# FriedFeid/Video-Depth-Anything

Measured on AMD Instinct MI355X. Metric: depth frames/sec at 32x518x518, ViT-L fp16, 1/2/4/8 MI355X, higher is better.
Workload: dtype fp16; 1 GPU; VideoDepthAnything.forward vitl 1x32x3x518x518 per GPU; encoder=vitl, frames_per_clip=32, H=518, W=518, clips_per_gpu=1, parallelism=clip-parallel dp1, ranks=1, depth_gather_to_rank0=False, hip_graph=False, clips_in_flight=2

## Files before the change

include/vda.h:

```cpp
#ifndef VDA_H
#define VDA_H

#include <stdint.h>

#ifdef __cplusplus
extern "C" {
#endif

enum {
  VDA_ACT_NONE = 0,
  VDA_ACT_GELU = 1,
  VDA_ACT_GEGLU = 2,
  VDA_ACT_RELU = 3,
  VDA_ACT_SWIGLU = 4
};

enum {
  VDA_STORE_ROWS = 0,
  VDA_STORE_PIXEL_SHUFFLE = 1
};

typedef struct vda_epilogue {
  const float* bias;
  const float* rowbias;
  int32_t rdiv, rmod;
  const float* gamma;
  const void* res;
  int64_t ldres;
  const void* res2;
  int64_t ldres2;
  int32_t act;
  int32_t store;
  int32_t ps_k, ps_cout, ps_hin, ps_win;
  const float* ln_stats;
  const float* ln_colsum;
  int32_t ln_parts;
  float ln_eps;
  float* stats_out;
  int32_t res2_h, res2_w;
  int32_t* sched;
  int32_t drop_period;
  const float* bias9;
} vda_epilogue;

const char* vda_version(void);
int64_t vda_epilogue_size(void);
const char* vda_last_error(void);

int vda_gemm(const void* x, int64_t ldx, const void* w, void* y, int64_t ldy,
             int32_t M, int32_t N, int32_t K, const vda_epilogue* epi, void* stream);
int vda_gemm_check(int64_t ldx, int64_t ldy, int32_t M, int32_t N, int32_t K, const vda_epilogue* epi);

int vda_conv2d(const void* x, const void* w, void* y, int32_t BT, int32_t H, int32_t W,
               int32_t Cin, int32_t Cout, int32_t ks, int32_t stride, int32_t pad,
               int32_t pre_relu, int32_t up_h, int32_t up_w, const vda_epilogue* epi,
               void* ws, int64_t ws_bytes, void* stream);
int64_t vda_conv2d_workspace(int32_t BT, int32_t H, int32_t W, int32_t Cin, int32_t Cout, int32_t ks,
                             int32_t stride, int32_t pad);
int vda_conv2d_res2_upsample_ok(int32_t BT, int32_t H, int32_t W, int32_t Cin, int32_t Cout, int32_t ks,
                                int32_t stride, int32_t pad);
int vda_conv2d_bias9_ok(int32_t BT, int32_t H, int32_t W, int32_t Cin, int32_t Cout, int32_t up_h, int32_t up_w);

int vda_subpixel_conv(const void* x, const void* w, const float* bias9, void* y, int32_t BT, int32_t h, int32_t w_,
                      int32_t Cin, int32_t Cout, int32_t s, void* ws, int64_t ws_bytes, void* stream);
int64_t vda_subpixel_conv_workspace(int32_t BT, int32_t h, int32_t w_, int32_t Cin, int32_t s);
int vda_subpixel_conv_check(int32_t BT, int32_t h, int32_t w_, int32_t Cin, int32_t Cout, int32_t s);

int vda_layernorm(const void* x, int64_t ldx, void* y, const float* gamma, const float* beta,
                  int32_t rows, int32_t C, float eps, int32_t skip_period, void* stream);

int vda_row_stats(const void* x, int64_t ldx, float* stats, int32_t rows, int32_t C, float eps,
                  void* stream);

int vda_groupnorm(const void* x, void* y, const float* gamma, const float* beta, int32_t F,
                  int32_t S, int32_t C, int32_t groups, float eps, float* ws, void* stream);
int64_t vda_groupnorm_workspace(int32_t F, int32_t S, int32_t C, int32_t groups);

int vda_groupnorm_linear(const void* x, const float* gamma, const float* beta, int32_t F, int32_t S,
                         int32_t C, int32_t groups, float eps, const void* w, const float* bias, void* y,
                         int32_t N, float* stats_out, void* ws, int64_t ws_bytes, void* stream);
int64_t vda_groupnorm_linear_workspace(int32_t F, int32_t S, int32_t C, int32_t groups, int32_t N);
int vda_groupnorm_linear_fused(int32_t C, int32_t groups, int32_t N);

int vda_spatial_attention(const void* qkv, void* out, int32_t B, int32_t N, int32_t H,
                          int32_t D, float scale, void* stream);

int vda_temporal_attention(const void* qkv, void* out, int32_t B, int32_t T, int32_t S,
                           int32_t H, int32_t D, float scale, float rope_theta, void* stream);

int vda_upsample_bilinear(const void* x, void* y, int32_t BT, int32_t H, int32_t W, int32_t C,
                          int32_t Ho, int32_t Wo, void* stream);

int vda_patch_im2col(const float* img, void* a, int32_t BT, int32_t H, int32_t W, int32_t Kp,
                     void* stream);

int vda_depth_head(const void* x, const void* w1, const float* b1, const float* w2,
                   const float* b2, float* depth, void* ws, int32_t BT, int32_t Hin, int32_t Win,
                   int32_t C, int32_t Ho, int32_t Wo, void* stream);
int64_t vda_depth_head_workspace(int32_t BT, int32_t Hin, int32_t Win, int32_t C, int32_t Ho, int32_t Wo);

int vda_preprocess_frames(const void* frames, float* out, int32_t N, int32_t h, int32_t w, int32_t H,
                          int32_t W, const float* mean, const float* std, void* stream);

int vda_depth_resize(const float* depth, float* out, int32_t N, int32_t H, int32_t W, int32_t ho,
                     int32_t wo, void* stream);

int64_t vda_scale_shift_workspace(int64_t n);
int vda_scale_shift(const float* pred, const float* target, const uint8_t* mask, int64_t n, double* sums,
                    float* ss, void* ws, int64_t ws_bytes, void* stream);

int vda_depth_align(const float* src, int32_t F, int32_t H, int32_t W, int32_t ho, int32_t wo, const float* ss,
                    int32_t clip, const float* pre, const float* w_pre, const float* w_post, float* out,
                    void* stream);

int64_t vda_depth_eval_workspace(int32_t F, int64_t S);
int vda_depth_eval_fit(const float* pred, const float* gt, const uint8_t* valid, int32_t F, int64_t S,
                       int32_t per_frame, double* sums, float* ss, void* ws, int64_t ws_bytes, void* stream);
int vda_depth_eval_metrics(const float* pred, const float* gt, const uint8_t* valid, int32_t F, int64_t S,
                           const float* ss, int32_t ss_per_frame, float max_depth, float* aligned,
                           double* frame_sums, double* total, void* ws, int64_t ws_bytes, void* stream);

enum {
  VDA_VIS_INDEX = 0,
  VDA_VIS_HWC = 1,
  VDA_VIS_PLANAR444 = 2,
  VDA_VIS_PLANAR420 = 3
};
int64_t vda_depth_range_workspace(int64_t n);
int vda_depth_range(const float* depth, int64_t n, float* range, void* ws, int64_t ws_bytes, void* stream);
int64_t vda_depth_colorize_bytes(int32_t F, int32_t H, int32_t W, int32_t layout);
int vda_depth_colorize(const float* depth, int32_t F, int32_t H, int32_t W, const float* range,
                       const uint8_t* lut, int32_t layout, uint8_t* out, void* stream);

enum {
  VDA_TILE_RGB = 0,
  VDA_TILE_DEPTH = 1,
  VDA_TILE_ERROR = 2,
  VDA_TILE_XT = 3
};
typedef struct vda_tile {
  int32_t kind;
  int32_t row, col;
  int32_t offset;
  int32_t frames;
  int32_t lut;
  const void* a;
  const float* b;
  const uint8_t* valid;
  const float* range;
} vda_tile;
int64_t vda_tile_size(void);
int64_t vda_depth_absdiff_range_workspace(int64_t n);
int vda_depth_absdiff_range(const float* a, const float* b, const uint8_t* valid, int64_t n, float* range, void* ws,
                            int64_t ws_bytes, void* stream);
int64_t vda_panel_compose_bytes(int32_t F, int32_t rows, int32_t cols, int32_t H, int32_t W, int32_t layout);
int vda_panel_compose(const vda_tile* tiles, int32_t ntiles, int32_t rows, int32_t cols, int32_t F, int32_t t0,
                      int32_t N, int32_t H, int32_t W, int32_t xstar, const uint8_t* lut0, const uint8_t* lut1,
                      int32_t layout, uint8_t* out, void* stream);

enum {
  VDA_YUV_420 = 0,
  VDA_YUV_422 = 1,
  VDA_YUV_444 = 2,
  VDA_YUV_MONO = 3
};
int vda_yuv_to_rgb(const uint8_t* src, int32_t N, int32_t h, int32_t w, int64_t frame_stride, int32_t chroma,
                   uint8_t* out, void* stream);
int64_t vda_preprocess_yuv_workspace(int32_t N, int32_t h, int32_t w, int32_t H, int32_t W);
int vda_preprocess_yuv(const uint8_t* src, int32_t N, int32_t h, int32_t w, int64_t frame_stride, int32_t chroma,
                       float* out, int32_t H, int32_t W, const float* mean, const float* stdv, void* ws,
                       int64_t ws_bytes, void* stream);
int32_t vda_resample_taps(int32_t in, int32_t out);
int vda_resample_tables(int32_t in, int32_t out, int32_t* k, int32_t* bounds);
int vda_yuv_downscale_ok(int32_t h, int32_t w, int32_t h2, int32_t w2);
int64_t vda_yuv_downscale_workspace(int32_t N, int32_t h, int32_t w, int32_t h2, int32_t w2);
int vda_yuv_downscale(const uint8_t* src, int32_t N, int32_t h, int32_t w, int64_t frame_stride, int32_t chroma,
                      const int32_t* kx, const int32_t* bx, const int32_t* ky, const int32_t* by, uint8_t* out,
                      int32_t h2, int32_t w2, void* ws, int64_t ws_bytes, void* stream);

int vda_gemm_f32(const float* x, int64_t ldx, const float* w, float* y, int64_t ldy,
                 int32_t M, int32_t N, int32_t K, const vda_epilogue* epi, void* stream);
int vda_conv2d_f32(const float* x, const float* w, float* y, int32_t BT, int32_t H, int32_t W,
                   int32_t Cin, int32_t Cout, int32_t ks, int32_t stride, int32_t pad,
                   int32_t pre_relu, const vda_epilogue* epi, void* stream);
int vda_layernorm_f32(const float* x, int64_t ldx, float* y, const float* gamma, const float* beta,
                      int32_t rows, int32_t C, float eps, int32_t skip_period, void* stream);
int vda_groupnorm_f32(const float* x, float* y, const float* gamma, const float* beta, int32_t F,
                      int32_t S, int32_t C, int32_t groups, float eps, void* stream);
int vda_spatial_attention_f32(const float* qkv, float* out, int32_t B, int32_t N, int32_t H,
                              int32_t D, float scale, void* stream);
int vda_temporal_attention_f32(const float* qkv, float* out, int32_t B, int32_t T, int32_t S,
                               int32_t H, int32_t D, float scale, float rope_theta, void* stream);
int vda_upsample_bilinear_f32(const float* x, float* y, int32_t BT, int32_t H, int32_t W, int32_t C,
                              int32_t Ho, int32_t Wo, void* stream);
int vda_patch_im2col_f32(const float* img, float* a, int32_t BT, int32_t H, int32_t W, int32_t Kp,
                         void* stream);
int vda_depth_head_f32(const float* x, const float* w1, const float* b1, const float* w2,
                       const float* b2, float* depth, float* ws_up, float* ws_mid, int32_t BT,
                       int32_t Hin, int32_t Win, int32_t C, int32_t Ho, int32_t Wo, void* stream);


#ifdef __cplusplus
}
#endif
#endif
```

include/vda_tune.h:

```cpp
#ifndef VDA_TUNE_H
#define VDA_TUNE_H
#include <stdint.h>
#ifdef __cplusplus
extern "C" {
#endif

int vda_debug_force_tile(int32_t cfg);
int vda_debug_gemm_sched(int32_t persist_blocks);
int vda_debug_strip_split(int32_t nsplit);
int vda_debug_hconv(int32_t mode);
int vda_debug_dconv(int32_t mode);
int vda_debug_oc1_src(int32_t mode);
int vda_debug_attn(int32_t temporal_direct);

#ifdef __cplusplus
}
#endif
#endif
```

video-depth-anything_amd/_lib.py:

```python
from __future__ import annotations

import ctypes
import os
from ctypes import c_float, c_int32, c_int64, c_void_p, POINTER

_HERE = os.path.dirname(os.path.abspath(__file__))
LIB_PATH = os.environ.get("VDA_LIB_OVERRIDE") or os.path.join(_HERE, "libvda.so")
TORCH_LIB_PATH = os.path.join(_HERE, "libvda_torch.so")
if os.environ.get("VDA_LIB_OVERRIDE"):
    _ov = os.path.join(os.path.dirname(os.path.abspath(os.environ["VDA_LIB_OVERRIDE"])), "libvda_torch.so")
    if os.path.exists(_ov):
        TORCH_LIB_PATH = _ov

EXPORTED = (
    "vda_version", "vda_epilogue_size", "vda_last_error", "vda_gemm", "vda_gemm_check", "vda_conv2d", "vda_conv2d_workspace",
    "vda_layernorm",
    "vda_conv2d_res2_upsample_ok", "vda_conv2d_bias9_ok",
    "vda_subpixel_conv", "vda_subpixel_conv_workspace", "vda_subpixel_conv_check",
    "vda_row_stats", "vda_groupnorm", "vda_groupnorm_workspace",
    "vda_groupnorm_linear", "vda_groupnorm_linear_workspace", "vda_groupnorm_linear_fused",
    "vda_spatial_attention", "vda_temporal_attention", "vda_upsample_bilinear", "vda_patch_im2col",
    "vda_depth_head", "vda_depth_head_workspace", "vda_preprocess_frames", "vda_depth_resize",
    "vda_scale_shift", "vda_scale_shift_workspace", "vda_depth_align",
    "vda_depth_eval_workspace", "vda_depth_eval_fit", "vda_depth_eval_metrics",
    "vda_depth_range_workspace", "vda_depth_range", "vda_depth_colorize_bytes", "vda_depth_colorize",
    "vda_tile_size", "vda_depth_absdiff_range_workspace", "vda_depth_absdiff_range", "vda_panel_compose_bytes",
    "vda_panel_compose",
    "vda_yuv_to_rgb", "vda_preprocess_yuv_workspace", "vda_preprocess_yuv",
    "vda_resample_taps", "vda_resample_tables", "vda_yuv_downscale_ok", "vda_yuv_downscale_workspace",
    "vda_yuv_downscale",
    "vda_gemm_f32", "vda_conv2d_f32", "vda_layernorm_f32", "vda_groupnorm_f32", "vda_spatial_attention_f32",
    "vda_temporal_attention_f32", "vda_upsample_bilinear_f32", "vda_patch_im2col_f32", "vda_depth_head_f32",
)
TUNE_EXPORTED = ("vda_debug_force_tile", "vda_debug_gemm_sched", "vda_debug_strip_split", "vda_debug_hconv",
                 "vda_debug_dconv", "vda_debug_attn", "vda_debug_oc1_src")
TUNE_LIB_PATH = os.path.join(os.path.dirname(_HERE), "build", "tune", "libvda.so")

ACT_NONE, ACT_GELU, ACT_GEGLU, ACT_RELU, ACT_SWIGLU = 0, 1, 2, 3, 4
STORE_ROWS, STORE_PIXEL_SHUFFLE = 0, 1
VIS_INDEX, VIS_HWC, VIS_PLANAR444, VIS_PLANAR420 = 0, 1, 2, 3
TILE_RGB, TILE_DEPTH, TILE_ERROR, TILE_XT = 0, 1, 2, 3
YUV_420, YUV_422, YUV_444, YUV_MONO = 0, 1, 2, 3


class VDAUnavailable(RuntimeError):
    pass


class VDAError(RuntimeError):
    pass


class Epilogue(ctypes.Structure):
    _fields_ = [
        ("bias", c_void_p), ("rowbias", c_void_p), ("rdiv", c_int32), ("rmod", c_int32),
        ("gamma", c_void_p), ("res", c_void_p), ("ldres", c_int64), ("res2", c_void_p),
        ("ldres2", c_int64), ("act", c_int32), ("store", c_int32), ("ps_k", c_int32),
        ("ps_cout", c_int32), ("ps_hin", c_int32), ("ps_win", c_int32),
        ("ln_stats", c_void_p), ("ln_colsum", c_void_p), ("ln_parts", c_int32), ("ln_eps", c_float),
        ("stats_out", c_void_p), ("res2_h", c_int32), ("res2_w", c_int32), ("sched", c_void_p),
        ("drop_period", c_int32), ("bias9", c_void_p),
    ]


class Tile(ctypes.Structure):
    _fields_ = [
        ("kind", c_int32), ("row", c_int32), ("col", c_int32), ("offset", c_int32), ("frames", c_int32),
        ("lut", c_int32), ("a", c_void_p), ("b", c_void_p), ("valid", c_void_p), ("range", c_void_p),
    ]


_lib = None
_load_error = None


def _declare(lib):
    P, I, L, F = c_void_p, c_int32, c_int64, c_float
    EP = POINTER(Epilogue)
    sig = {
        "vda_version": ([], ctypes.c_char_p),
        "vda_epilogue_size": ([], L),
        "vda_last_error": ([], ctypes.c_char_p),
        "vda_gemm": ([P, L, P, P, L, I, I, I, EP, P], I),
        "vda_gemm_check": ([L, L, I, I, I, EP], I),
        "vda_conv2d": ([P, P, P, I, I, I, I, I, I, I, I, I, I, I, EP, P, L, P], I),
        "vda_conv2d_workspace": ([I, I, I, I, I, I, I, I], L),
        "vda_conv2d_res2_upsample_ok": ([I, I, I, I, I, I, I, I], I),
        "vda_conv2d_bias9_ok": ([I, I, I, I, I, I, I], I),
        "vda_subpixel_conv": ([P, P, P, P, I, I, I, I, I, I, P, L, P], I),
        "vda_subpixel_conv_workspace": ([I, I, I, I, I], L),
        "vda_subpixel_conv_check": ([I, I, I, I, I, I], I),
        "vda_layernorm": ([P, L, P, P, P, I, I, F, I, P], I),
        "vda_row_stats": ([P, L, P, I, I, F, P], I),
        "vda_groupnorm": ([P, P, P, P, I, I, I, I, F, P, P], I),
        "vda_groupnorm_workspace": ([I, I, I, I], L),
        "vda_groupnorm_linear": ([P, P, P, I, I, I, I, F, P, P, P, I, P, P, L, P], I),
        "vda_groupnorm_linear_workspace": ([I, I, I, I, I], L),
        "vda_groupnorm_linear_fused": ([I, I, I], I),
        "vda_spatial_attention": ([P, P, I, I, I, I, F, P], I),
        "vda_temporal_attention": ([P, P, I, I, I, I, I, F, F, P], I),
        "vda_upsample_bilinear": ([P, P, I, I, I, I, I, I, P], I),
        "vda_patch_im2col": ([P, P, I, I, I, I, P], I),
        "vda_depth_head": ([P, P, P, P, P, P, P, I, I, I, I, I, I, P], I),
        "vda_depth_head_workspace": ([I, I, I, I, I, I], L),
        "vda_preprocess_frames": ([P, P, I, I, I, I, I, POINTER(F), POINTER(F), P], I),
        "vda_depth_resize": ([P, P, I, I, I, I, I, P], I),
        "vda_scale_shift_workspace": ([L], L),
        "vda_scale_shift": ([P, P, P, L, P, P, P, L, P], I),
        "vda_depth_align": ([P, I, I, I, I, I, P, I, P, POINTER(F), POINTER(F), P, P], I),
        "vda_depth_eval_workspace": ([I, L], L),
        "vda_depth_eval_fit": ([P, P, P, I, L, I, P, P, P, L, P], I),
        "vda_depth_eval_metrics": ([P, P, P, I, L, P, I, F, P, P, P, P, L, P], I),
        "vda_depth_range_workspace": ([L], L),
        "vda_depth_range": ([P, L, P, P, L, P], I),
        "vda_depth_colorize_bytes": ([I, I, I, I], L),
        "vda_depth_colorize": ([P, I, I, I, P, P, I, P, P], I),
        "vda_tile_size": ([], L),
        "vda_depth_absdiff_range_workspace": ([L], L),
        "vda_depth_absdiff_range": ([P, P, P, L, P, P, L, P], I),
        "vda_panel_compose_bytes": ([I, I, I, I, I, I], L),
        "vda_panel_compose": ([POINTER(Tile), I, I, I, I, I, I, I, I, I, P, P, I, P, P], I),
        "vda_yuv_to_rgb": ([P, I, I, I, L, I, P, P], I),
        "vda_preprocess_yuv_workspace": ([I, I, I, I, I], L),
        "vda_preprocess_yuv": ([P, I, I, I, L, I, P, I, I, POINTER(F), POINTER(F), P, L, P], I),
        "vda_resample_taps": ([I, I], I),
        "vda_resample_tables": ([I, I, P, P], I),
        "vda_yuv_downscale_ok": ([I, I, I, I], I),
        "vda_yuv_downscale_workspace": ([I, I, I, I, I], L),
        "vda_yuv_downscale": ([P, I, I, I, L, I, P, P, P, P, P, I, I, P, L, P], I),
        "vda_gemm_f32": ([P, L, P, P, L, I, I, I, EP, P], I),
        "vda_conv2d_f32": ([P, P, P, I, I, I, I, I, I, I, I, I, EP, P], I),
        "vda_layernorm_f32": ([P, L, P, P, P, I, I, F, I, P], I),
        "vda_groupnorm_f32": ([P, P, P, P, I, I, I, I, F, P], I),
        "vda_spatial_attention_f32": ([P, P, I, I, I, I, F, P], I),
        "vda_temporal_attention_f32": ([P, P, I, I, I, I, I, F, F, P], I),
        "vda_upsample_bilinear_f32": ([P, P, I, I, I, I, I, I, P], I),
        "vda_patch_im2col_f32": ([P, P, I, I, I, I, P], I),
        "vda_depth_head_f32": ([P, P, P, P, P, P, P, P, I, I, I, I, I, I, P], I),
        "vda_debug_force_tile": ([I], I),
        "vda_debug_gemm_sched": ([I], I),
        "vda_debug_strip_split": ([I], I),
        "vda_debug_hconv": ([I], I),
        "vda_debug_dconv": ([I], I),
        "vda_debug_attn": ([I], I),
        "vda_debug_oc1_src": ([I], I),
    }
    for name, (args, res) in sig.items():
        if name.startswith("vda_debug_") and not hasattr(lib, name):
            continue
        fn = getattr(lib, name)
        fn.argtypes = args
        fn.restype = res


def lib():
    global _lib, _load_error
    if _lib is not None:
        return _lib
    if _load_error is not None:
        raise VDAUnavailable(_load_error)
    if not os.path.exists(LIB_PATH):
        _load_error = f"libvda.so not found at {LIB_PATH}; run `make` (or __graft_entry__.build())"
        raise VDAUnavailable(_load_error)
    try:
        l = ctypes.CDLL(LIB_PATH)
        _declare(l)
        if l.vda_epilogue_size() != ctypes.sizeof(Epilogue):
            raise OSError(f"vda_epilogue is {l.vda_epilogue_size()} bytes in the library, {ctypes.sizeof(Epilogue)} "
                          f"in _lib.Epilogue: rebuild libvda.so or update the mirror")
        if l.vda_tile_size() != ctypes.sizeof(Tile):
            raise OSError(f"vda_tile is {l.vda_tile_size()} bytes in the library, {ctypes.sizeof(Tile)} in _lib.Tile: "
                          f"rebuild libvda.so or update the mirror")
    except OSError as e:
        _load_error = f"failed to load {LIB_PATH}: {e}"
        raise VDAUnavailable(_load_error) from e
    _lib = l
    return _lib


_torch_ops = None


def torch_ops():
    global _torch_ops
    if _torch_ops is not None:
        return _torch_ops
    lib()
    if not os.path.exists(TORCH_LIB_PATH):
        raise VDAUnavailable(f"libvda_torch.so not found at {TORCH_LIB_PATH}; run `make` (or __graft_entry__.build())")
    import torch
    try:
        torch.ops.load_library(TORCH_LIB_PATH)
    except OSError as e:
        raise VDAUnavailable(f"failed to load {TORCH_LIB_PATH}: {e}") from e
    _torch_ops = torch.ops.vda
    return _torch_ops


def check(rc: int, what: str):
    if rc != 0:
        msg = lib().vda_last_error().decode(errors="replace")
        raise VDAError(f"{what} failed (rc={rc}): {msg}")
```

video-depth-anything_amd/csrc/vda_hconv.hip:

```cpp
#include "vda_internal.h"
#include "vda_halo.h"
#include <type_traits>

namespace {

constexpr int HC_TR = 8, HC_TC = 32;
constexpr int HC_PC = HC_TC + 2;
constexpr int HC_NPIX = (HC_TR + 2) * HC_PC;
constexpr int HC_PSTR = 9;
constexpr int HC_PP = (HC_NPIX * HC_PSTR + 63) / 64;
constexpr int HC_PSLOT = HC_PP * 512;
constexpr int HC_PPW = (HC_PP + 7) / 8;
static_assert(HC_PP % 8 == 0, "the wait_vmcnt counts assume every wave issues HC_PPW patch pieces");
constexpr int HC_BK = 64;
constexpr int HC_HALF = 128 * HC_BK;
constexpr int HC_WBUF = 2 * HC_HALF;
static_assert(HC_PPW <= 9, "patch pieces are issued in the first steps of a slab");

__device__ __attribute__((aligned(64))) uint4 g_hc_zero[4];

#ifdef VDA_TS
__device__ unsigned long long g_hts[8192][6];
#define HTS(k) (hts[k] = __builtin_amdgcn_s_memrealtime())
#else
#define HTS(k) ((void)0)
#endif

__device__ __forceinline__ int hc_swz(int row, int chunk) { return row * HC_BK + ((chunk ^ ((row >> 1) & 7)) << 3); }

struct HconvArgs {
  const h16* x;
  const h16* w;
  h16* y;
  const float* bias;
  const h16* res;
  const h16* res2;
  int r2h, r2w;
  int H, W, Cin, relu_out;
  int tiles_x, tiles_y, ntiles;
};

template <bool PRE>
__global__ __launch_bounds__(512) void hconv256_kernel(HconvArgs a) {
  __shared__ __attribute__((aligned(1024))) h16 smem[2 * HC_WBUF + 2 * HC_PSLOT];
#ifdef VDA_TS
  unsigned long long hts[6];
#endif
  HTS(0);
  h16* const wsm = smem;
  h16* const psm = smem + 2 * HC_WBUF;

  int tid;
  asm volatile("v_mov_b32 %0, %1" : "=v"(tid) : "v"((int)threadIdx.x));
  const int lane = tid & 63;
  const int wave = __builtin_amdgcn_readfirstlane(tid >> 6);
  const int wm = wave & 1, wn = wave >> 1;

  int bt, y0, x0;
  {
    const int bid = blockIdx.x, nwg = a.ntiles;
    const int xcd = bid & 7, q = nwg >> 3, r = nwg & 7;
    const int t = (xcd < r ? xcd * (q + 1) : r * (q + 1) + (xcd - r) * q) + (bid >> 3);
    const int tx = t % a.tiles_x;
    const int rr = t / a.tiles_x;
    y0 = (rr % a.tiles_y) * HC_TR;
    x0 = tx * HC_TC;
    bt = rr / a.tiles_y;
  }
  const int H = a.H, W = a.W, Cin = a.Cin;
  const int K = 9 * Cin;
  const int nslab = Cin / 64;
  const int NK = 9 * nslab;
  const h16* xf0 = a.x + (long)bt * H * W * Cin;

  int poff[HC_PPW];
#pragma unroll
  for (int j = 0; j < HC_PPW; ++j) {
    const int q = wave + 8 * j;
    const int sl = q * 64 + lane;
    const int p = sl / HC_PSTR, cd = sl - p * HC_PSTR;
    const int pr = p / HC_PC, pc = p - pr * HC_PC;
    const int iy = y0 - 1 + pr, ix = x0 - 1 + pc;
    poff[j] = (q < HC_PP && p < HC_NPIX && cd < 8 && (unsigned)iy < (unsigned)H && (unsigned)ix < (unsigned)W)
                  ? (iy * W + ix) * Cin + cd * 8
                  : -1;
  }
  uint64_t zpa = (uint64_t)(uintptr_t)g_hc_zero;
  asm volatile("" : "+s"(zpa));
  const void* const zero = (const void*)(uintptr_t)zpa;
  auto patch_piece = [&](int slab, int j) {
    const int q = wave + 8 * j;
    if (q < HC_PP) {
      const void* src = poff[j] >= 0 ? (const void*)(xf0 + poff[j] + slab * 64) : zero;
      glds16(src, psm + (slab & 1) * HC_PSLOT + q * 512);
    }
  };

  auto wr_of = [&](int i) { return (wave >> 2) * 64 + i * 32 + (wave & 3) * 8 + (lane >> 3); };
  const int kch0 = ((lane & 7) ^ ((((wave & 1) << 3 | (lane >> 3)) >> 1) & 7)) * 8;
  const __amdgpu_buffer_rsrc_t wrs =
      __builtin_amdgcn_make_buffer_rsrc((void*)a.w, (short)0, (int)(256L * K * 2), 0x00020000);
  unsigned wvo[2][2];
#pragma unroll
  for (int i = 0; i < 2; ++i)
#pragma unroll
    for (int hh = 0; hh < 2; ++hh) wvo[hh][i] = (unsigned)(((hh * 128 + wr_of(i)) * K + kch0) * 2);
  auto koff = [&](int kt) {
    const int slab = kt / 9, tap = kt - slab * 9;
    return (tap * Cin + slab * 64) * 2;
  };
  auto stage_w = [&](int kt, int buf, int i) {
    const int so = koff(kt);
#pragma unroll
    for (int hh = 0; hh < 2; ++hh)
      __builtin_amdgcn_raw_ptr_buffer_load_lds(
          wrs, (VDA_LDS void*)(wsm + buf * HC_WBUF + hh * HC_HALF + (wr_of(i) - (lane >> 3)) * HC_BK), 16,
          (int)wvo[hh][i], so, 0, 0);
  };

  f4 acc[4][8];
#pragma unroll
  for (int i = 0; i < 4; ++i)
#pragma unroll
    for (int j = 0; j < 8; ++j) acc[i][j] = f4{0.f, 0.f, 0.f, 0.f};
  f4 bias_r[4];
#pragma unroll
  for (int i = 0; i < 4; ++i)
    bias_r[i] = a.bias ? *reinterpret_cast<const f4*>(a.bias + wn * 64 + i * 16 + (lane >> 4) * 4) : f4{0.f, 0.f, 0.f, 0.f};

#pragma unroll
  for (int j = 0; j < HC_PPW; ++j) patch_piece(0, j);
  stage_w(0, 0, 0);
  stage_w(0, 0, 1);
  if (NK > 1) {
    stage_w(1, 1, 1);
    wait_vmcnt<2>();
  } else {
    wait_vmcnt<0>();
  }
  __builtin_amdgcn_s_barrier();
  static_assert(HC_PP * 64 == 6 * 512, "relu pass: two passes of 3 slots per thread cover the patch exactly");
  auto relu_pass = [&](int slot, int part) {
    h8* ps = reinterpret_cast<h8*>(psm + slot * HC_PSLOT) + tid + 512 * 3 * part;
    h8 v[3];
#pragma unroll
    for (int k = 0; k < 3; ++k) v[k] = ps[512 * k];
#pragma unroll
    for (int k = 0; k < 3; ++k) ps[512 * k] = relu8(v[k]);
  };
  if (PRE) {
    relu_pass(0, 0);
    relu_pass(0, 1);
    asm volatile("s_waitcnt lgkmcnt(0)" ::: "memory");
    __builtin_amdgcn_s_barrier();
  }
  HTS(1);
  const bool lagging = wave >= 4;
  if (lagging) __builtin_amdgcn_s_barrier();

  const int frow = lane & 15, fchunk = lane >> 4;
  const int woff = (wn >> 1) * HC_HALF;
  const int wrow0 = (wn & 1) * 64;
  h8 xf[4][2], wf[2][2];
  const unsigned xlane = (unsigned)(((wm * 4 * HC_PC + frow) * HC_PSTR + fchunk) * 16);
  auto load_x = [&](const h16* ps, int toff, int qm) {
    unsigned tb;
    asm volatile("s_mov_b32 %0, %1" : "=s"(tb) : "s"((unsigned)((uintptr_t)(VDA_LDS const h16*)ps) + (unsigned)(toff * HC_PSTR * 16)));
    const VDA_LDS char* xb = reinterpret_cast<const VDA_LDS char*>((uintptr_t)(tb + xlane));
#pragma unroll
    for (int j = 0; j < 4; ++j)
#pragma unroll
      for (int ks = 0; ks < 2; ++ks)
        xf[j][ks] = *reinterpret_cast<const VDA_LDS h8*>(
            xb + ((qm * 2 + (j >> 1)) * HC_PC + (j & 1) * 16) * HC_PSTR * 16 + ks * 64);
  };
  auto load_w = [&](const h16* base, int qn) {
#pragma unroll
    for (int i = 0; i < 2; ++i)
#pragma unroll
      for (int ks = 0; ks < 2; ++ks)
        wf[i][ks] = *reinterpret_cast<const h8*>(&base[woff + hc_swz(wrow0 + qn * 32 + i * 16 + frow, ks * 4 + fchunk)]);
  };
  auto mma = [&](int qm, int qn) {
    __builtin_amdgcn_s_barrier();
    asm volatile("s_waitcnt lgkmcnt(0)" ::: "memory");
    __builtin_amdgcn_sched_barrier(0);
    __builtin_amdgcn_s_setprio(1);
#pragma unroll
    for (int ks = 0; ks < 2; ++ks)
#pragma unroll
      for (int i = 0; i < 2; ++i)
#pragma unroll
        for (int j = 0; j < 4; ++j)
          acc[qn * 2 + i][qm * 4 + j] = mfma16(wf[i][ks], xf[j][ks], acc[qn * 2 + i][qm * 4 + j]);
    __builtin_amdgcn_s_setprio(0);
    __builtin_amdgcn_sched_barrier(0);
    __builtin_amdgcn_s_barrier();
  };

  for (int slab = 0; slab < nslab; ++slab) {
    const h16* ps = psm + (slab & 1) * HC_PSLOT;
    const bool nxt = slab + 1 < nslab;
    auto step = [&](auto tap_c) {
      constexpr int tap = decltype(tap_c)::value;
      constexpr int toff = (tap / 3) * HC_PC + (tap % 3);
      const int kt = slab * 9 + tap;
      const int cb = kt & 1, nb = cb ^ 1;
      const h16* base = wsm + cb * HC_WBUF;
      const bool more1 = kt + 1 < NK, more2 = kt + 2 < NK;
      load_x(ps, toff, 0);
      load_w(base, 0);
      if (tap < HC_PPW && nxt) patch_piece(slab + 1, tap < HC_PPW ? tap : 0);
      mma(0, 0);
      load_w(base, 1);
      if (more1) stage_w(kt + 1, nb, 0);
      if (PRE && tap >= 7 && nxt) relu_pass((slab + 1) & 1, tap >= 7 ? tap - 7 : 0);
      mma(0, 1);
      load_x(ps, toff, 1);
      mma(1, 1);
      load_w(base, 0);
      if (more2) {
        stage_w(kt + 2, cb, 1);
        wait_vmcnt<2>();
      } else {
        wait_vmcnt<0>();
      }
      mma(1, 0);
    };
    step(std::integral_constant<int, 0>{}); step(std::integral_constant<int, 1>{});
    step(std::integral_constant<int, 2>{}); step(std::integral_constant<int, 3>{});
    step(std::integral_constant<int, 4>{}); step(std::integral_constant<int, 5>{});
    step(std::integral_constant<int, 6>{}); step(std::integral_constant<int, 7>{});
    step(std::integral_constant<int, 8>{});
  }
  if (!lagging) __builtin_amdgcn_s_barrier();
  HTS(2);
  __syncthreads();

  const int q = tid & 31, row0 = tid >> 5;
  const h16* l0 = smem + row0 * 256 + ((2 * q) ^ row0) * 4;
  const h16* l1 = smem + row0 * 256 + ((2 * q + 1) ^ row0) * 4;
  const long fbytes = (long)H * W * 512;
  const long fbase = (long)bt * H * W * 256;
  auto rsrc = [&](const h16* p) {
    return __builtin_amdgcn_make_buffer_rsrc((void*)(p + fbase), (short)0, (int)fbytes, 0x00020000);
  };
  const __amdgpu_buffer_rsrc_t ry = rsrc(a.y);
  auto voff = [&](int it) {
    const int yy = y0 + (it >> 1), xx = x0 + row0 + 16 * (it & 1);
    return (yy < H && xx < W) ? (unsigned)(((yy * W + xx) * 256 + q * 8) * 2) : 0x80000000u;
  };
  const bool up2 = a.r2h > 0;
  const h16* pres2 = up2 ? nullptr : a.res2;
  const int nres = (a.res ? 1 : 0) + (pres2 ? 1 : 0);
  const h16* r1p = a.res ? a.res : pres2;
  const __amdgpu_buffer_rsrc_t rr1 = rsrc(r1p ? r1p : a.y);
  const __amdgpu_buffer_rsrc_t rr2 = rsrc(pres2 ? pres2 : a.y);
  const __amdgpu_buffer_rsrc_t rs2 = __builtin_amdgcn_make_buffer_rsrc(
      (void*)((up2 ? a.res2 : a.y) + (up2 ? (long)bt * a.r2h * a.r2w * 256 : fbase)), (short)0,
      up2 ? (int)((long)a.r2h * a.r2w * 512) : (int)fbytes, 0x00020000);
  const float usy = a.r2h > 0 ? ac_scale(a.r2h, H) : 0.f, usx = a.r2w > 0 ? ac_scale(a.r2w, W) : 0.f;
  auto up_load = [&](int it, h8* t4, float& wx, float& wy) {
    const int yy = min(y0 + (it >> 1), H - 1), xx = min(x0 + row0 + 16 * (it & 1), W - 1);
    int sy0, sy1, sx0, sx1;
    ac_coord(yy, a.r2h, usy, sy0, sy1, wy);
    ac_coord(xx, a.r2w, usx, sx0, sx1, wx);
    const unsigned r0 = (unsigned)(sy0 * a.r2w), r1 = (unsigned)(sy1 * a.r2w), c8 = (unsigned)q * 16u;
    t4[0] = __builtin_bit_cast(h8, __builtin_amdgcn_raw_buffer_load_b128(rs2, (r0 + sx0) * 512u + c8, 0, 0));
    t4[1] = __builtin_bit_cast(h8, __builtin_amdgcn_raw_buffer_load_b128(rs2, (r0 + sx1) * 512u + c8, 0, 0));
    t4[2] = __builtin_bit_cast(h8, __builtin_amdgcn_raw_buffer_load_b128(rs2, (r1 + sx0) * 512u + c8, 0, 0));
    t4[3] = __builtin_bit_cast(h8, __builtin_amdgcn_raw_buffer_load_b128(rs2, (r1 + sx1) * 512u + c8, 0, 0));
  };
  constexpr int UPD = 2;
  h8 u4[UPD][4];
  float uwx[UPD], uwy[UPD];
  if (up2) {
#pragma unroll
    for (int it = 0; it < UPD; ++it) up_load(it, u4[it], uwx[it], uwy[it]);
  }
  constexpr int PD = 4;
  h8 q1[PD], q2[PD];
  if (nres >= 1) {
#pragma unroll
    for (int it = 0; it < PD; ++it) q1[it] = __builtin_bit_cast(h8, __builtin_amdgcn_raw_buffer_load_b128(rr1, voff(it), 0, 0));
  }
  if (nres >= 2) {
#pragma unroll
    for (int it = 0; it < PD; ++it) q2[it] = __builtin_bit_cast(h8, __builtin_amdgcn_raw_buffer_load_b128(rr2, voff(it), 0, 0));
  }
  const int mcol = lane & 15, nq = (lane >> 4) * 4;
#pragma unroll
  for (int i = 0; i < 4; ++i) {
    const int col = wn * 64 + i * 16 + nq;
    const f4 bv = bias_r[i];
#pragma unroll
    for (int j = 0; j < 8; ++j) {
      const int ml = wm * 128 + j * 16 + mcol;
      f4 v = acc[i][j] + bv;
      if (a.relu_out) {
#pragma unroll
        for (int r = 0; r < 4; ++r) v[r] = fmaxf(v[r], 0.f);
      }
      typedef float f2v __attribute__((ext_vector_type(2)));
      const h2 lo = __builtin_convertvector(f2v{v[0], v[1]}, h2);
      const h2 hi = __builtin_convertvector(f2v{v[2], v[3]}, h2);
      const int u = (col >> 2) ^ (ml & 15);
      *reinterpret_cast<uint2*>(&smem[ml * 256 + u * 4]) =
          make_uint2(__builtin_bit_cast(unsigned, lo), __builtin_bit_cast(unsigned, hi));
    }
  }
  __syncthreads();
  HTS(3);
#pragma unroll
  for (int it = 0; it < 16; ++it) {
    const uint2 lo = *reinterpret_cast<const uint2*>(l0 + it * 16 * 256);
    const uint2 hi = *reinterpret_cast<const uint2*>(l1 + it * 16 * 256);
    h8 t = __builtin_bit_cast(h8, make_uint4(lo.x, lo.y, hi.x, hi.y));
    const unsigned vo = voff(it);
    if (nres >= 1) {
      t += q1[it % PD];
      if (it + PD < 16) q1[it % PD] = __builtin_bit_cast(h8, __builtin_amdgcn_raw_buffer_load_b128(rr1, voff(it + PD), 0, 0));
    }
    if (nres >= 2) {
      t += q2[it % PD];
      if (it + PD < 16) q2[it % PD] = __builtin_bit_cast(h8, __builtin_amdgcn_raw_buffer_load_b128(rr2, voff(it + PD), 0, 0));
    }
    if (up2) {
      const int sl = it % UPD;
      t += bilerp8(u4[sl][0], u4[sl][1], u4[sl][2], u4[sl][3], uwx[sl], uwy[sl]);
      if (it + UPD < 16) up_load(it + UPD, u4[sl], uwx[sl], uwy[sl]);
    }
    __builtin_amdgcn_raw_buffer_store_b128(__builtin_bit_cast(u32x4, t), ry, vo, 0, 2);
  }
#ifdef VDA_TS
  HTS(4);
  asm volatile("s_waitcnt vmcnt(0)" ::: "memory");
  HTS(5);
  if (tid == 0 && blockIdx.x < 8192)
    for (int k = 0; k < 6; ++k) g_hts[blockIdx.x][k] = hts[k];
#endif
}

}

VDA_KNOB(int, g_hconv_mode, -1);

bool vda_conv_hconv_serves(int BT, int H, int W, int Cin, int Cout) {
  if (Cout != 256 || Cin % 64 != 0 || Cin <= 0 || g_hconv_mode == 0) return false;
  if ((long)BT * ((H + HC_TR - 1) / HC_TR) * ((W + HC_TC - 1) / HC_TC) > 0x7fffffffL) return false;
  if ((long)H * W * Cin >= (1L << 31) || (long)H * W * 512 >= (1L << 31)) return false;
  if (g_hconv_mode == 1) return true;
  return (long)H * W >= 64L * 64L;
}

int vda_conv_hconv(const void* x, const void* w, void* y, const float* bias, int relu_out, int pre_relu,
                   const void* res, const void* res2, int res2_h, int res2_w, int BT, int H, int W, int Cin, int Cout,
                   hipStream_t st) {
  if (!vda_conv_hconv_serves(BT, H, W, Cin, Cout)) return 1;
  HconvArgs a{};
  a.x = (const h16*)x; a.w = (const h16*)w; a.y = (h16*)y; a.bias = bias;
  a.res = (const h16*)res; a.res2 = (const h16*)res2;
  a.r2h = res2 && res2_h > 0 && res2_w > 0 ? res2_h : 0;
  a.r2w = a.r2h > 0 ? res2_w : 0;
  a.H = H; a.W = W; a.Cin = Cin; a.relu_out = relu_out;
  a.tiles_x = (W + HC_TC - 1) / HC_TC;
  a.tiles_y = (H + HC_TR - 1) / HC_TR;
  a.ntiles = BT * a.tiles_x * a.tiles_y;
  if (pre_relu)
    hipLaunchKernelGGL(hconv256_kernel<true>, dim3(a.ntiles), dim3(512), 0, st, a);
  else
    hipLaunchKernelGGL(hconv256_kernel<false>, dim3(a.ntiles), dim3(512), 0, st, a);
  VDA_LAUNCH_CHECK();
  return 0;
}

#ifdef VDA_TS
extern "C" int vda_debug_hconv_timestamps(void* host) {
  return (int)hipMemcpyFromSymbol(host, HIP_SYMBOL(g_hts), sizeof(g_hts), 0, hipMemcpyDeviceToHost);
}
#endif
#ifdef VDA_TUNING
extern "C" int vda_debug_hconv(int32_t mode) {
  g_hconv_mode = mode;
  return 0;
}
#endif
```

Baseline: 741.8 frames/s.

## Template the 256-out 3x3 conv on tile shape and pick the fewest-tile shape

The hconv256 kernel becomes a template over its output tile shape, with 8x32, 10x25 and 16x16 on a menu. A host-side chooser picks the shape that covers the feature map with the fewest tiles, which cuts edge padding waste on the 74/148/296-wide DPT maps. Tiles whose width is not a multiple of 16 need a padded LDS patch pitch, per-fragment row-crossing address fixups (bfe/mad) and a remapped epilogue pixel index. The cost is extra ALU work in the fragment loads and some extra LDS pitch on those shapes.

```diff
diff --git a/include/vda.h b/include/vda.h
--- a/include/vda.h
+++ b/include/vda.h
@@ -60,6 +60,7 @@
 int vda_conv2d_res2_upsample_ok(int32_t BT, int32_t H, int32_t W, int32_t Cin, int32_t Cout, int32_t ks,
                                 int32_t stride, int32_t pad);
 int vda_conv2d_bias9_ok(int32_t BT, int32_t H, int32_t W, int32_t Cin, int32_t Cout, int32_t up_h, int32_t up_w);
+int vda_hconv_tile_shape(int32_t H, int32_t W, int32_t* tr, int32_t* tc);
 
 int vda_subpixel_conv(const void* x, const void* w, const float* bias9, void* y, int32_t BT, int32_t h, int32_t w_,
                       int32_t Cin, int32_t Cout, int32_t s, void* ws, int64_t ws_bytes, void* stream);
diff --git a/include/vda_tune.h b/include/vda_tune.h
--- a/include/vda_tune.h
+++ b/include/vda_tune.h
@@ -9,6 +9,7 @@
 int vda_debug_gemm_sched(int32_t persist_blocks);
 int vda_debug_strip_split(int32_t nsplit);
 int vda_debug_hconv(int32_t mode);
+int vda_debug_hconv_tile(int32_t k);
 int vda_debug_dconv(int32_t mode);
 int vda_debug_oc1_src(int32_t mode);
 int vda_debug_attn(int32_t temporal_direct);
diff --git a/video-depth-anything_amd/_lib.py b/video-depth-anything_amd/_lib.py
--- a/video-depth-anything_amd/_lib.py
+++ b/video-depth-anything_amd/_lib.py
@@ -15,7 +15,7 @@
 EXPORTED = (
     "vda_version", "vda_epilogue_size", "vda_last_error", "vda_gemm", "vda_gemm_check", "vda_conv2d", "vda_conv2d_workspace",
     "vda_layernorm",
-    "vda_conv2d_res2_upsample_ok", "vda_conv2d_bias9_ok",
+    "vda_conv2d_res2_upsample_ok", "vda_conv2d_bias9_ok", "vda_hconv_tile_shape",
     "vda_subpixel_conv", "vda_subpixel_conv_workspace", "vda_subpixel_conv_check",
     "vda_row_stats", "vda_groupnorm", "vda_groupnorm_workspace",
     "vda_groupnorm_linear", "vda_groupnorm_linear_workspace", "vda_groupnorm_linear_fused",
@@ -33,7 +33,7 @@
     "vda_temporal_attention_f32", "vda_upsample_bilinear_f32", "vda_patch_im2col_f32", "vda_depth_head_f32",
 )
 TUNE_EXPORTED = ("vda_debug_force_tile", "vda_debug_gemm_sched", "vda_debug_strip_split", "vda_debug_hconv",
-                 "vda_debug_dconv", "vda_debug_attn", "vda_debug_oc1_src")
+                 "vda_debug_dconv", "vda_debug_attn", "vda_debug_oc1_src", "vda_debug_hconv_tile")
 TUNE_LIB_PATH = os.path.join(os.path.dirname(_HERE), "build", "tune", "libvda.so")
 
 ACT_NONE, ACT_GELU, ACT_GEGLU, ACT_RELU, ACT_SWIGLU = 0, 1, 2, 3, 4
@@ -74,7 +74,7 @@
 _load_error = None
 
 
-def _declare(lib):
+def _declare(lib, older=False):
     P, I, L, F = c_void_p, c_int32, c_int64, c_float
     EP = POINTER(Epilogue)
     sig = {
@@ -87,6 +87,7 @@
         "vda_conv2d_workspace": ([I, I, I, I, I, I, I, I], L),
         "vda_conv2d_res2_upsample_ok": ([I, I, I, I, I, I, I, I], I),
         "vda_conv2d_bias9_ok": ([I, I, I, I, I, I, I], I),
+        "vda_hconv_tile_shape": ([I, I, POINTER(I), POINTER(I)], I),
         "vda_subpixel_conv": ([P, P, P, P, I, I, I, I, I, I, P, L, P], I),
         "vda_subpixel_conv_workspace": ([I, I, I, I, I], L),
         "vda_subpixel_conv_check": ([I, I, I, I, I, I], I),
@@ -141,12 +142,15 @@
         "vda_debug_gemm_sched": ([I], I),
         "vda_debug_strip_split": ([I], I),
         "vda_debug_hconv": ([I], I),
+        "vda_debug_hconv_tile": ([I], I),
         "vda_debug_dconv": ([I], I),
         "vda_debug_attn": ([I], I),
         "vda_debug_oc1_src": ([I], I),
     }
     for name, (args, res) in sig.items():
         if name.startswith("vda_debug_") and not hasattr(lib, name):
+            continue
+        if older and not hasattr(lib, name):
             continue
         fn = getattr(lib, name)
         fn.argtypes = args
@@ -164,7 +168,7 @@
         raise VDAUnavailable(_load_error)
     try:
         l = ctypes.CDLL(LIB_PATH)
-        _declare(l)
+        _declare(l, older=bool(os.environ.get("VDA_LIB_OVERRIDE")))
         if l.vda_epilogue_size() != ctypes.sizeof(Epilogue):
             raise OSError(f"vda_epilogue is {l.vda_epilogue_size()} bytes in the library, {ctypes.sizeof(Epilogue)} "
                           f"in _lib.Epilogue: rebuild libvda.so or update the mirror")
diff --git a/video-depth-anything_amd/csrc/vda_hconv.hip b/video-depth-anything_amd/csrc/vda_hconv.hip
--- a/video-depth-anything_amd/csrc/vda_hconv.hip
+++ b/video-depth-anything_amd/csrc/vda_hconv.hip
@@ -4,9 +4,7 @@
 
 namespace {
 
-constexpr int HC_TR = 8, HC_TC = 32;
-constexpr int HC_PC = HC_TC + 2;
-constexpr int HC_NPIX = (HC_TR + 2) * HC_PC;
+constexpr int HC_NPIX = 340;
 constexpr int HC_PSTR = 9;
 constexpr int HC_PP = (HC_NPIX * HC_PSTR + 63) / 64;
 constexpr int HC_PSLOT = HC_PP * 512;
@@ -25,6 +23,25 @@
 #else
 #define HTS(k) ((void)0)
 #endif
+
+template <int TR, int TC>
+struct HcShape {
+  static_assert(TC >= 16, "a 16-pixel fragment crosses at most one row end");
+  static_assert(TR * TC <= 256, "one MFMA column per tile pixel");
+  static_assert((TR + 2) * (TC + 2) <= HC_NPIX, "the patch fits the slot");
+  static constexpr int PC = TC + 2;
+  static constexpr bool straight = TC % 16 == 0 && 128 % TC == 0;
+  static constexpr int RPAD = straight ? 0 : 1;
+  static constexpr int RPITCH = PC * HC_PSTR + RPAD;
+  static constexpr int ROWSH = 2 * HC_PSTR + RPAD;
+  static constexpr int pslot(int p) { return p * HC_PSTR + (p / TC) * ROWSH; }
+  static_assert((TR + 2) * RPITCH <= HC_PP * 64, "the padded patch fits the slot");
+  static_assert(pslot(255) + 2 * RPITCH + 2 * HC_PSTR + 8 <= HC_PP * 64,
+                "the last (dead) column's last tap reads inside the slot");
+};
+
+constexpr int HC_NMENU = 3;
+constexpr int HC_MENU[HC_NMENU][2] = {{8, 32}, {10, 25}, {16, 16}};
 
 __device__ __forceinline__ int hc_swz(int row, int chunk) { return row * HC_BK + ((chunk ^ ((row >> 1) & 7)) << 3); }
 
@@ -40,8 +57,9 @@
   int tiles_x, tiles_y, ntiles;
 };
 
-template <bool PRE>
+template <bool PRE, int TR, int TC>
 __global__ __launch_bounds__(512) void hconv256_kernel(HconvArgs a) {
+  using S = HcShape<TR, TC>;
   __shared__ __attribute__((aligned(1024))) h16 smem[2 * HC_WBUF + 2 * HC_PSLOT];
 #ifdef VDA_TS
   unsigned long long hts[6];
@@ -63,8 +81,8 @@
     const int t = (xcd < r ? xcd * (q + 1) : r * (q + 1) + (xcd - r) * q) + (bid >> 3);
     const int tx = t % a.tiles_x;
     const int rr = t / a.tiles_x;
-    y0 = (rr % a.tiles_y) * HC_TR;
-    x0 = tx * HC_TC;
+    y0 = (rr % a.tiles_y) * TR;
+    x0 = tx * TC;
     bt = rr / a.tiles_y;
   }
   const int H = a.H, W = a.W, Cin = a.Cin;
@@ -78,12 +96,22 @@
   for (int j = 0; j < HC_PPW; ++j) {
     const int q = wave + 8 * j;
     const int sl = q * 64 + lane;
-    const int p = sl / HC_PSTR, cd = sl - p * HC_PSTR;
-    const int pr = p / HC_PC, pc = p - pr * HC_PC;
-    const int iy = y0 - 1 + pr, ix = x0 - 1 + pc;
-    poff[j] = (q < HC_PP && p < HC_NPIX && cd < 8 && (unsigned)iy < (unsigned)H && (unsigned)ix < (unsigned)W)
-                  ? (iy * W + ix) * Cin + cd * 8
-                  : -1;
+    if constexpr (S::RPAD == 0) {
+      const int p = sl / HC_PSTR, cd = sl - p * HC_PSTR;
+      const int pr = p / S::PC, pc = p - pr * S::PC;
+      const int iy = y0 - 1 + pr, ix = x0 - 1 + pc;
+      poff[j] = (q < HC_PP && p < (TR + 2) * S::PC && cd < 8 && (unsigned)iy < (unsigned)H && (unsigned)ix < (unsigned)W)
+                    ? (iy * W + ix) * Cin + cd * 8
+                    : -1;
+    } else {
+      const int pr = (int)((unsigned)sl / (unsigned)S::RPITCH);
+      const unsigned ws = (unsigned)(sl - pr * S::RPITCH);
+      const int pc = (int)(ws / (unsigned)HC_PSTR), cd = (int)ws - pc * HC_PSTR;
+      const int iy = y0 - 1 + pr, ix = x0 - 1 + pc;
+      poff[j] = (q < HC_PP && pr < TR + 2 && pc < S::PC && cd < 8 && (unsigned)iy < (unsigned)H && (unsigned)ix < (unsigned)W)
+                    ? (iy * W + ix) * Cin + cd * 8
+                    : -1;
+    }
   }
   uint64_t zpa = (uint64_t)(uintptr_t)g_hc_zero;
   asm volatile("" : "+s"(zpa));
@@ -124,9 +152,11 @@
 #pragma unroll
     for (int j = 0; j < 8; ++j) acc[i][j] = f4{0.f, 0.f, 0.f, 0.f};
   f4 bias_r[4];
-#pragma unroll
-  for (int i = 0; i < 4; ++i)
-    bias_r[i] = a.bias ? *reinterpret_cast<const f4*>(a.bias + wn * 64 + i * 16 + (lane >> 4) * 4) : f4{0.f, 0.f, 0.f, 0.f};
+  if constexpr (S::RPAD == 0) {
+  #pragma unroll
+    for (int i = 0; i < 4; ++i)
+      bias_r[i] = a.bias ? *reinterpret_cast<const f4*>(a.bias + wn * 64 + i * 16 + (lane >> 4) * 4) : f4{0.f, 0.f, 0.f, 0.f};
+  }
 
 #pragma unroll
   for (int j = 0; j < HC_PPW; ++j) patch_piece(0, j);
@@ -162,17 +192,33 @@
   const int woff = (wn >> 1) * HC_HALF;
   const int wrow0 = (wn & 1) * 64;
   h8 xf[4][2], wf[2][2];
-  const unsigned xlane = (unsigned)(((wm * 4 * HC_PC + frow) * HC_PSTR + fchunk) * 16);
-  auto load_x = [&](const h16* ps, int toff, int qm) {
+  const unsigned xlane = S::RPAD == 0 ? (unsigned)(((wm * (S::pslot(128) / HC_PSTR) + frow) * HC_PSTR + fchunk) * 16)
+                                     : (unsigned)((wm * S::pslot(128) + frow * HC_PSTR + fchunk) * 16);
+  unsigned xrows = 0;
+  if constexpr (!S::straight) {
+#pragma unroll
+    for (int k = 0; k < 8; ++k)
+      xrows |= (unsigned)((128 * wm + 16 * k + frow) / TC - (16 * k) / TC - wm * (128 / TC)) << (2 * k);
+  }
+  auto load_x = [&](const h16* ps, int toff, auto qm_c) {
+    constexpr int qm = decltype(qm_c)::value;
     unsigned tb;
-    asm volatile("s_mov_b32 %0, %1" : "=s"(tb) : "s"((unsigned)((uintptr_t)(VDA_LDS const h16*)ps) + (unsigned)(toff * HC_PSTR * 16)));
-    const VDA_LDS char* xb = reinterpret_cast<const VDA_LDS char*>((uintptr_t)(tb + xlane));
-#pragma unroll
-    for (int j = 0; j < 4; ++j)
+    asm volatile("s_mov_b32 %0, %1" : "=s"(tb) : "s"((unsigned)((uintptr_t)(VDA_LDS const h16*)ps) + (unsigned)(toff * 16)));
+    const unsigned xq = tb + xlane;
+#pragma unroll
+    for (int j = 0; j < 4; ++j) {
+      const int k = qm * 4 + j;
+      unsigned xa = xq;
+      if constexpr (!S::straight) {
+        asm volatile("v_bfe_u32 %0, %1, %2, 2\n\tv_mad_u32_u24 %0, %0, %3, %4"
+                     : "=&v"(xa)
+                     : "v"(xrows), "i"(2 * k), "s"((unsigned)(S::ROWSH * 16)), "v"(xq));
+      }
+      const VDA_LDS char* xb = reinterpret_cast<const VDA_LDS char*>((uintptr_t)xa);
 #pragma unroll
       for (int ks = 0; ks < 2; ++ks)
-        xf[j][ks] = *reinterpret_cast<const VDA_LDS h8*>(
-            xb + ((qm * 2 + (j >> 1)) * HC_PC + (j & 1) * 16) * HC_PSTR * 16 + ks * 64);
+        xf[j][ks] = *reinterpret_cast<const VDA_LDS h8*>(xb + S::pslot(16 * k) * 16 + ks * 64);
+    }
   };
   auto load_w = [&](const h16* base, int qn) {
 #pragma unroll
@@ -203,12 +249,12 @@
     const bool nxt = slab + 1 < nslab;
     auto step = [&](auto tap_c) {
       constexpr int tap = decltype(tap_c)::value;
-      constexpr int toff = (tap / 3) * HC_PC + (tap % 3);
+      constexpr int toff = (tap / 3) * S::RPITCH + (tap % 3) * HC_PSTR;
       const int kt = slab * 9 + tap;
       const int cb = kt & 1, nb = cb ^ 1;
       const h16* base = wsm + cb * HC_WBUF;
       const bool more1 = kt + 1 < NK, more2 = kt + 2 < NK;
-      load_x(ps, toff, 0);
+      load_x(ps, toff, std::integral_constant<int, 0>{});
       load_w(base, 0);
       if (tap < HC_PPW && nxt) patch_piece(slab + 1, tap < HC_PPW ? tap : 0);
       mma(0, 0);
@@ -216,7 +262,7 @@
       if (more1) stage_w(kt + 1, nb, 0);
       if (PRE && tap >= 7 && nxt) relu_pass((slab + 1) & 1, tap >= 7 ? tap - 7 : 0);
       mma(0, 1);
-      load_x(ps, toff, 1);
+      load_x(ps, toff, std::integral_constant<int, 1>{});
       mma(1, 1);
       load_w(base, 0);
       if (more2) {
@@ -235,9 +281,27 @@
   }
   if (!lagging) __builtin_amdgcn_s_barrier();
   HTS(2);
+  if constexpr (S::RPAD != 0) {
+  #pragma unroll
+    for (int i = 0; i < 4; ++i)
+      bias_r[i] = a.bias ? *reinterpret_cast<const f4*>(a.bias + wn * 64 + i * 16 + (lane >> 4) * 4) : f4{0.f, 0.f, 0.f, 0.f};
+  }
   __syncthreads();
 
   const int q = tid & 31, row0 = tid >> 5;
+  auto tile_px = [&](int it, int& py, int& pc) {
+    const int r = (16 * it) / TC, c = (16 * it) % TC;
+    if constexpr (TC % 16 == 0) {
+      py = r;
+      pc = c;
+      return TR * TC == 256 || 16 * it < TR * TC;
+    } else {
+      const bool cross = row0 + c >= TC;
+      py = r + (cross ? 1 : 0);
+      pc = c - (cross ? TC : 0);
+      return TR * TC == 256 || row0 + 16 * it < TR * TC;
+    }
+  };
   const h16* l0 = smem + row0 * 256 + ((2 * q) ^ row0) * 4;
   const h16* l1 = smem + row0 * 256 + ((2 * q + 1) ^ row0) * 4;
   const long fbytes = (long)H * W * 512;
@@ -247,8 +311,10 @@
   };
   const __amdgpu_buffer_rsrc_t ry = rsrc(a.y);
   auto voff = [&](int it) {
-    const int yy = y0 + (it >> 1), xx = x0 + row0 + 16 * (it & 1);
-    return (yy < H && xx < W) ? (unsigned)(((yy * W + xx) * 256 + q * 8) * 2) : 0x80000000u;
+    int py, pc;
+    const bool live = tile_px(it, py, pc);
+    const int yy = y0 + py, xx = x0 + row0 + pc;
+    return (live && yy < H && xx < W) ? (unsigned)(((yy * W + xx) * 256 + q * 8) * 2) : 0x80000000u;
   };
   const bool up2 = a.r2h > 0;
   const h16* pres2 = up2 ? nullptr : a.res2;
@@ -261,7 +327,9 @@
       up2 ? (int)((long)a.r2h * a.r2w * 512) : (int)fbytes, 0x00020000);
   const float usy = a.r2h > 0 ? ac_scale(a.r2h, H) : 0.f, usx = a.r2w > 0 ? ac_scale(a.r2w, W) : 0.f;
   auto up_load = [&](int it, h8* t4, float& wx, float& wy) {
-    const int yy = min(y0 + (it >> 1), H - 1), xx = min(x0 + row0 + 16 * (it & 1), W - 1);
+    int py, pc;
+    tile_px(it, py, pc);
+    const int yy = min(y0 + py, H - 1), xx = min(x0 + row0 + pc, W - 1);
     int sy0, sy1, sx0, sx1;
     ac_coord(yy, a.r2h, usy, sy0, sy1, wy);
     ac_coord(xx, a.r2w, usx, sx0, sx1, wx);
@@ -344,13 +412,48 @@
 }
 
 VDA_KNOB(int, g_hconv_mode, -1);
+VDA_KNOB(int, g_hconv_tile, 0);
+
+static long hc_tiles(int m, int H, int W) {
+  const int tr = HC_MENU[m][0], tc = HC_MENU[m][1];
+  return (long)((H + tr - 1) / tr) * ((W + tc - 1) / tc);
+}
+
+static int hc_auto_shape(int H, int W) {
+  int best = 0;
+  for (int m = 1; m < HC_NMENU; ++m) {
+    const long t = hc_tiles(m, H, W), tb = hc_tiles(best, H, W);
+    if (t < tb || (t == tb && best != 0 && HC_MENU[m][0] * HC_MENU[m][1] > HC_MENU[best][0] * HC_MENU[best][1])) best = m;
+  }
+  return best;
+}
+
+static int hc_shape(int H, int W) { return g_hconv_tile >= 1 ? g_hconv_tile - 1 : hc_auto_shape(H, W); }
+
+extern "C" int vda_hconv_tile_shape(int32_t H, int32_t W, int32_t* tr, int32_t* tc) {
+  VDA_CHECK_ARG(tr && tc, "null pointer");
+  VDA_CHECK_ARG(H > 0 && W > 0, "empty map");
+  const int m = hc_auto_shape(H, W);
+  *tr = HC_MENU[m][0];
+  *tc = HC_MENU[m][1];
+  return 0;
+}
 
 bool vda_conv_hconv_serves(int BT, int H, int W, int Cin, int Cout) {
   if (Cout != 256 || Cin % 64 != 0 || Cin <= 0 || g_hconv_mode == 0) return false;
-  if ((long)BT * ((H + HC_TR - 1) / HC_TR) * ((W + HC_TC - 1) / HC_TC) > 0x7fffffffL) return false;
+  if (H <= 0 || W <= 0 || (long)BT * hc_tiles(hc_shape(H, W), H, W) > 0x7fffffffL) return false;
   if ((long)H * W * Cin >= (1L << 31) || (long)H * W * 512 >= (1L << 31)) return false;
   if (g_hconv_mode == 1) return true;
   return (long)H * W >= 64L * 64L;
+}
+
+template <int M>
+static void hc_launch(const HconvArgs& a, int pre_relu, hipStream_t st) {
+  constexpr int TR = HC_MENU[M][0], TC = HC_MENU[M][1];
+  if (pre_relu)
+    hipLaunchKernelGGL((hconv256_kernel<true, TR, TC>), dim3(a.ntiles), dim3(512), 0, st, a);
+  else
+    hipLaunchKernelGGL((hconv256_kernel<false, TR, TC>), dim3(a.ntiles), dim3(512), 0, st, a);
 }
 
 int vda_conv_hconv(const void* x, const void* w, void* y, const float* bias, int relu_out, int pre_relu,
@@ -363,13 +466,16 @@
   a.r2h = res2 && res2_h > 0 && res2_w > 0 ? res2_h : 0;
   a.r2w = a.r2h > 0 ? res2_w : 0;
   a.H = H; a.W = W; a.Cin = Cin; a.relu_out = relu_out;
-  a.tiles_x = (W + HC_TC - 1) / HC_TC;
-  a.tiles_y = (H + HC_TR - 1) / HC_TR;
+  const int m = hc_shape(H, W);
+  a.tiles_x = (W + HC_MENU[m][1] - 1) / HC_MENU[m][1];
+  a.tiles_y = (H + HC_MENU[m][0] - 1) / HC_MENU[m][0];
   a.ntiles = BT * a.tiles_x * a.tiles_y;
-  if (pre_relu)
-    hipLaunchKernelGGL(hconv256_kernel<true>, dim3(a.ntiles), dim3(512), 0, st, a);
-  else
-    hipLaunchKernelGGL(hconv256_kernel<false>, dim3(a.ntiles), dim3(512), 0, st, a);
+  static_assert(HC_NMENU == 3, "one case per menu entry");
+  switch (m) {
+    case 0: hc_launch<0>(a, pre_relu, st); break;
+    case 1: hc_launch<1>(a, pre_relu, st); break;
+    default: hc_launch<2>(a, pre_relu, st); break;
+  }
   VDA_LAUNCH_CHECK();
   return 0;
 }
@@ -384,4 +490,9 @@
   g_hconv_mode = mode;
   return 0;
 }
+extern "C" int vda_debug_hconv_tile(int32_t k) {
+  if (k < 0 || k > HC_NMENU) return -22;
+  g_hconv_tile = k;
+  return 0;
+}
 #endif
```

New measurement: 742.8 frames/s, median of 6. About the same (+0.1%).
